# CityU-AIM-Group/SimT

Hardware: AMD Instinct MI355X
Metric: training images/sec at 768x768, DeepLabv2-R101+SimT (higher is better)
Workload: dtype bf16; 1 GPU; DeepLabv2-ResNet101 + SimT(C=19,K=3) full training iteration, batch=4/GPU, 768x768, bf16, 1xMI355X; global_batch=4, inputs=resident in HBM (see h2d_inclusive of a --full run for the PCIe-inclusive rate)

## Files before the change

### simt_amd/csrc/head_expand.hip

```cpp
#include "common.h"

struct TapArgs {
  const void* src;
  const float* bias;
  void* dst;
  int B, H, W, Q, QP, lds, ldd, ntaps;
  long M;
  short dy[SIMT_MAX_TAPS], dx[SIMT_MAX_TAPS];
};

__global__ __launch_bounds__(256) void tap_gather_sum_kernel(TapArgs a) {
  const int nq = a.QP >> 2;
  const long total = a.M * nq;
  const float* P = (const float*)a.src;
  float* y = (float*)a.dst;
  for (long idx = (long)blockIdx.x * blockDim.x + threadIdx.x; idx < total; idx += (long)gridDim.x * blockDim.x) {
    const int q = (int)(idx % nq);
    const long m = idx / nq;
    const int ox = (int)(m % a.W);
    const long t2 = m / a.W;
    const int oy = (int)(t2 % a.H);
    float4 acc = make_float4(0.f, 0.f, 0.f, 0.f);
    if (a.bias) {
      const int c = q * 4;
      acc.x = c + 0 < a.Q ? a.bias[c + 0] : 0.f;
      acc.y = c + 1 < a.Q ? a.bias[c + 1] : 0.f;
      acc.z = c + 2 < a.Q ? a.bias[c + 2] : 0.f;
      acc.w = c + 3 < a.Q ? a.bias[c + 3] : 0.f;
    }
    for (int t = 0; t < a.ntaps; ++t) {
      const int iy = oy + a.dy[t], ix = ox + a.dx[t];
      if (iy < 0 || iy >= a.H || ix < 0 || ix >= a.W) continue;
      const float4 v = *(const float4*)(P + (m + (long)a.dy[t] * a.W + a.dx[t]) * a.lds + t * a.QP + q * 4);
      acc.x += v.x; acc.y += v.y; acc.z += v.z; acc.w += v.w;
    }
    *(float4*)(y + m * a.ldd + q * 4) = acc;
  }
}

__global__ __launch_bounds__(256) void tap_scatter_kernel(TapArgs a) {
  const int ng = a.QP >> 3;
  const long total = a.M * a.ntaps * ng;
  const bf16_t* d = (const bf16_t*)a.src;
  bf16_t* G = (bf16_t*)a.dst;
  for (long idx = (long)blockIdx.x * blockDim.x + threadIdx.x; idx < total; idx += (long)gridDim.x * blockDim.x) {
    const int g = (int)(idx % ng);
    long r = idx / ng;
    const int t = (int)(r % a.ntaps);
    const long m = r / a.ntaps;
    const int ox = (int)(m % a.W);
    const int oy = (int)((m / a.W) % a.H);
    const int iy = oy - a.dy[t], ix = ox - a.dx[t];
    uint4 v = make_uint4(0u, 0u, 0u, 0u);
    if (iy >= 0 && iy < a.H && ix >= 0 && ix < a.W)
      v = *(const uint4*)(d + (m - ((long)a.dy[t] * a.W + a.dx[t])) * a.lds + g * 8);
    st_out16(G + m * a.ldd + t * a.QP + g * 8, v);
  }
}

static int tap_grid(long total) {
  long g = (total + 255) / 256;
  if (g > 256 * 16) g = 256 * 16;
  return (int)(g < 1 ? 1 : g);
}

extern "C" int simt_tap_gather_sum(const simt_tap_desc* d, simt_stream_t stream) {
  SIMT_CHECK(d && d->src && d->dst && d->ntaps >= 1 && d->ntaps <= SIMT_MAX_TAPS);
  SIMT_CHECK(d->QP % 4 == 0 && d->lds % 4 == 0 && d->ldd % 4 == 0 && d->QP <= d->ldd && d->ntaps * d->QP <= d->lds);
  TapArgs a;
  a.src = d->src; a.bias = d->bias; a.dst = d->dst; a.B = d->B; a.H = d->H; a.W = d->W; a.Q = d->Q; a.QP = d->QP;
  a.lds = d->lds; a.ldd = d->ldd; a.ntaps = d->ntaps; a.M = (long)d->B * d->H * d->W;
  for (int i = 0; i < SIMT_MAX_TAPS; ++i) { a.dy[i] = d->dy[i]; a.dx[i] = d->dx[i]; }
  hipLaunchKernelGGL(tap_gather_sum_kernel, dim3(tap_grid(a.M * (a.QP / 4))), dim3(256), 0, (hipStream_t)stream, a);
  SIMT_LAUNCH_CHECK();
  return SIMT_OK;
}

extern "C" int simt_tap_scatter(const simt_tap_desc* d, simt_stream_t stream) {
  SIMT_CHECK(d && d->src && d->dst && d->ntaps >= 1 && d->ntaps <= SIMT_MAX_TAPS);
  SIMT_CHECK(d->QP % 8 == 0 && d->lds % 8 == 0 && d->ldd % 8 == 0 && d->QP <= d->lds && d->ntaps * d->QP <= d->ldd);
  TapArgs a;
  a.src = d->src; a.bias = nullptr; a.dst = d->dst; a.B = d->B; a.H = d->H; a.W = d->W; a.Q = d->Q; a.QP = d->QP;
  a.lds = d->lds; a.ldd = d->ldd; a.ntaps = d->ntaps; a.M = (long)d->B * d->H * d->W;
  for (int i = 0; i < SIMT_MAX_TAPS; ++i) { a.dy[i] = d->dy[i]; a.dx[i] = d->dx[i]; }
  hipLaunchKernelGGL(tap_scatter_kernel, dim3(tap_grid(a.M * a.ntaps * (a.QP / 8))), dim3(256), 0, (hipStream_t)stream, a);
  SIMT_LAUNCH_CHECK();
  return SIMT_OK;
}
```

### simt_amd/step.py

```python
import ctypes as C
import math
import os

import numpy as np
import torch

from . import _lib as L
from . import ops
from . import trace
from .ema import EmaMixin
from .ema_teacher import TeacherMixin
from .engine import LaunchList, TrunkPlan, multi_heads, side_stream
from .online_labels import OnlineLabelMixin, check_balanced, check_settings
from .train_state import TrainStateMixin, state_sha256


class Hyper:

    def __init__(self, num_classes=19, open_classes=15, th_high=0.8, th_low=0.2, lambda_seg=0.1, lambda_place=0.1,
                 lambda_convex=0.5, lambda_volume=0.1, lambda_anchor=0.5, iter_size=1, lr=2.5e-4, lr_T=2.5e-4,
                 momentum=0.9, weight_decay=5e-4, power=0.9, num_steps=250000, skip_unapplied_grads=False):
        self.__dict__.update(locals())
        del self.__dict__["self"]


def lr_poly(base_lr, it, max_iter, power):
    return base_lr * ((1 - float(it) / max_iter) ** power)


def optim_listing(names, layers_root=("layer3", "layer4"), head_prefixes=("layer5", "layer6", "layer5_1", "layer6_1")):
    g0, g1 = {}, {}
    for n in names:
        root = n.split(".")[0]
        if root in layers_root:
            depth = len(n.split(".")) - 1
            g0[n] = depth
        elif root in head_prefixes:
            g1[n] = 1
    return g0, g1


def check_views(tr, teacher_image, fix_item, n):
    if not tr.teacher_view:
        if teacher_image is not None or fix_item is not None:
            raise ValueError("step(): teacher_image / fix_item need a trainer built with teacher_view=True")
        return [None] * n, [None] * n
    if teacher_image is None:
        raise ValueError("step(): this trainer was built with teacher_view=True and needs teacher_image (the frozen model's view)")
    teachers = list(teacher_image) if isinstance(teacher_image, (list, tuple)) else [teacher_image]
    maps = list(fix_item) if isinstance(fix_item, (list, tuple)) else [fix_item] * (n if fix_item is None else 1)
    if len(teachers) != n or len(maps) != n:
        raise ValueError(f"step() needs {n} teacher_image(s) and fix_item(s) (hp.iter_size), got {len(teachers)} and {len(maps)}")
    for t in teachers:
        if tuple(t.shape) != (tr.B, 3, tr.H, tr.W):
            raise ValueError(f"teacher_image of shape {tuple(t.shape)}, expected {(tr.B, 3, tr.H, tr.W)}")
    for m in maps:
        if m is not None and (tuple(m.shape) != (tr.B, tr.H, tr.W) or m.dtype != torch.uint8):
            raise ValueError(f"fix_item of shape {tuple(m.shape)} and dtype {m.dtype}, expected {(tr.B, tr.H, tr.W)} uint8")
    return teachers, maps


class SimTTrainer(TrainStateMixin, EmaMixin, TeacherMixin):
    def __init__(self, state, fixed_state, ntm1, ntm2, hp, class_dist, B, H, W, *, dtype=torch.bfloat16, device="cuda:0",
                 openset=True, process_group=None, w_init=None, layers=None, ema_decay=None, ema_teacher_every=None, teacher_view=False):
        self.hp, self.B, self.H, self.W, self.dtype = hp, B, H, W, dtype
        self.teacher_view = bool(teacher_view)
        dev = self.dev = torch.device(device)
        self.pg = process_group
        Cn, K = hp.num_classes, hp.open_classes
        self.C, self.Q = Cn, Cn + K
        f32 = torch.float32
        self.params = {k: v.detach().to(dev, f32 if v.dtype != torch.long else torch.long).clone() for k, v in state.items()}
        self.fixed_params = {k: v.detach().to(dev, f32 if v.dtype != torch.long else torch.long).clone()
                             for k, v in fixed_state.items()}
        self.frozen_sha256 = state_sha256(self.fixed_params)
        kw = {"layers": layers} if layers is not None else {}
        self.plan = TrunkPlan(self.params, B, H, W, multi_heads(Cn, K, openset), dtype=dtype, train=True,
                              grads_from_layer=3 if getattr(hp, "skip_unapplied_grads", False) else 0,
                              data_parallel=process_group is not None, **kw)
        self.fixed = TrunkPlan(self.fixed_params, B, H, W, multi_heads(Cn, 0, False), dtype=dtype, train=False,
                               stem_from=None if self.teacher_view else self.plan,
                               data_parallel=process_group is not None, **kw)
        assert self.plan.fwd_list.items[0].tag in ("simt_stem7_fwd", "simt_im2col_stem")
        assert self.plan.fwd_list.items[0].tag == "simt_im2col_stem" or self.plan.stem_desc.nsets == (1 if self.teacher_view else 2)
        assert not self.teacher_view or self.fixed.fwd_list.items[0].tag == self.plan.fwd_list.items[0].tag
        self._fwd_rest = LaunchList()
        self._fwd_rest.items = self.plan.fwd_list.items[1:]
        h, w = self.plan.heads[1].h, self.plan.heads[1].w
        self.h, self.w = h, w
        Q = self.Q
        self.ntm = [ntm1.detach().to(dev, f32).clone(), ntm2.detach().to(dev, f32).clone()]
        self._xchg = torch.zeros(16 + 2 * Q * Cn, device=dev)
        self._ntm_grad_flat = self._xchg[16:].view(2, Q, Cn)
        self.ntm_grad = [self._ntm_grad_flat[0], self._ntm_grad_flat[1]]
        self.ntm_m = [torch.zeros(Q, Cn, device=dev) for _ in range(2)]
        self.ntm_v = [torch.zeros(Q, Cn, device=dev) for _ in range(2)]
        wi = w_init if w_init is not None else torch.full((Q, Q), 1.0 / (Q - 1.0))
        self.wraw = [wi.detach().to(dev, f32).clone() for _ in range(2)]
        self.w_m = [torch.zeros(Q, Q, device=dev) for _ in range(2)]
        self.w_v = [torch.zeros(Q, Q, device=dev) for _ in range(2)]
        self.T = [torch.zeros(Q, Cn, device=dev) for _ in range(2)]
        self.cd = torch.as_tensor(np.asarray(class_dist), dtype=f32).to(dev)
        self.inner_steps = 10
        lib = L.load()
        self.nblk = lib.simt_head_nblk(B, H, W)
        self.part = torch.zeros(self.nblk, lib.simt_head_part_floats(Q, Cn), device=dev)
        self.keys = torch.zeros(lib.simt_head_keys_count(), device=dev, dtype=torch.int64)
        self.hout = torch.zeros(lib.simt_head_hout_floats(Q, Cn), device=dev)
        self.lout = self._xchg[:16]
        self._bad_reported = 0
        self.QP = ops.round_up(Q, 8)
        self.g1 = torch.zeros(2, B, H, w, self.QP, device=dev)
        self.ldf = self.fixed.ldp["x2"]
        self.fixp = torch.zeros(B * h * w, self.ldf, device=dev)
        self.label = torch.zeros(B, H, W, device=dev, dtype=torch.int64)
        hd = L.HeadDesc()
        p1, p2 = self.plan.out["x1"], self.plan.out["x2"]
        hd.pred1, hd.pred2, hd.fixp, hd.label = p1.data_ptr(), p2.data_ptr(), self.fixp.data_ptr(), self.label.data_ptr()
        hd.T1, hd.T2 = self.T[0].data_ptr(), self.T[1].data_ptr()
        hd.part, hd.keys, hd.hout, hd.g1 = self.part.data_ptr(), self.keys.data_ptr(), self.hout.data_ptr(), self.g1.data_ptr()
        hd.dpred1_f32, hd.dpred2_f32 = None, None
        d1, d2 = self.plan.dlogits["x1"], self.plan.dlogits["x2"]
        hd.dpred1_t, hd.dpred2_t = d1.data_ptr(), d2.data_ptr()
        hd.B, hd.h, hd.w, hd.H, hd.W, hd.C, hd.Q = B, h, w, H, W, Cn, Q
        hd.ldp, hd.ldf, hd.QP, hd.ld_f32, hd.ld_t = self.plan.ldp["x1"], self.ldf, self.QP, 0, d1.shape[1]
        hd.grad_dtype = ops.dt_code(dtype)
        hd.th_high, hd.th_low, hd.lambda_seg, hd.lambda_place = hp.th_high, hp.th_low, hp.lambda_seg, hp.lambda_place
        hd.gscale = 1.0 / hp.iter_size
        self.conf_label = torch.full((B, H, W), 255, device=dev, dtype=torch.uint8)
        hd.conf_out = self.conf_label.data_ptr()
        self._label_ws = torch.full((B, H, W), 255, device=dev, dtype=torch.uint8)
        hd.label_ws = self._label_ws.data_ptr()
        self.head_desc = hd
        self.fix_item = torch.zeros(B, H, W, device=dev, dtype=torch.uint8) if self.teacher_view else None
        self._fix_item_ptr = None
        ni = L.NtmInnerDesc()
        for k in range(2):
            ni.ntm[k], ni.w[k], ni.ntm_grad[k] = self.ntm[k].data_ptr(), self.wraw[k].data_ptr(), self.ntm_grad[k].data_ptr()
            ni.w_m[k], ni.w_v[k], ni.T_out[k] = self.w_m[k].data_ptr(), self.w_v[k].data_ptr(), self.T[k].data_ptr()
        ni.class_dist, ni.Q, ni.C, ni.steps = self.cd.data_ptr(), Q, Cn, self.inner_steps
        ni.beta1, ni.beta2, ni.eps = 0.9, 0.999, 1e-8
        self._skip_word = getattr(self.plan, "fbn_err", None)
        if self._skip_word is not None:
            ni.skip_if = self._skip_word.data_ptr()
        self.inner_desc = ni
        npd = L.NtmPostDesc()
        for k in range(2):
            npd.ntm[k], npd.w[k], npd.ntm_grad[k] = self.ntm[k].data_ptr(), self.wraw[k].data_ptr(), self.ntm_grad[k].data_ptr()
        npd.class_dist, npd.hout, npd.lout, npd.Q, npd.C = self.cd.data_ptr(), self.hout.data_ptr(), self.lout.data_ptr(), Q, Cn
        npd.lambda_seg, npd.lambda_convex, npd.lambda_volume = hp.lambda_seg, hp.lambda_convex, hp.lambda_volume
        npd.lambda_anchor, npd.gscale = hp.lambda_anchor, 1.0 / hp.iter_size
        self.post_desc = npd
        self._build_sgd()
        self.it_done = 0
        self._init_ema(ema_decay)
        self._init_teacher(ema_teacher_every)
        applied = [n for n in self.sgd_names if self.plan.grad_ready.get(n, 0) > 0]
        self._ev_post = None
        self._early_cut = max(self.plan.grad_ready[n] for n in applied) if applied else None
        if self._early_cut is not None:
            blk = min((m for m in self.plan.bwd_marks.values() if m[1] >= self._early_cut), key=lambda m: m[1], default=None)
            if blk is not None and blk[3] is not None:
                later = [c for c in sorted(set(self.plan.grad_ready.values())) if c >= blk[1]]
                self._early_cut = later[0] if later else None
        self._early_sgd = (os.environ.get("SIMT_EARLY_SGD", "1") != "0" and self._early_cut is not None
                           and hp.iter_size == 1 and self._early_cut < len(self.plan.bwd_list.items))
        self._pack_applied = self.plan.pack_subset(self.sgd_names) if self._early_sgd else None
        self._grad_acc = torch.zeros_like(self.plan.flat_grad) if hp.iter_size > 1 else None
        self.reducer = None
        if self.pg is not None:
            from .dp import BucketReducer, make_buckets
            order, sizes, end = self.exchange_table()
            be = int(float(os.environ.get("SIMT_DP_BUCKET_MB", "0")) * (1 << 18)) or self.BUCKET_ELEMS
            buckets = make_buckets(order, sizes, self.plan.grad_ready, bucket_elems=be)
            self.reducer = BucketReducer(self.plan.flat_grad[:end], buckets, group=self.pg, extra=[self._xchg[12:]])
            self.reducer.total_launches = len(self.plan.bwd_list.items)

    BUCKET_ELEMS = 8 << 20

    def exchange_table(self):
        sizes = {n: k for n, (_o, k) in self.plan.grad_offsets.items()}
        applied = set(self.sgd_names)
        order = [n for n in self.plan.grad_order if n in applied and self.plan.grad_ready.get(n, 0) > 0]
        assert order == self.plan.grad_order[:len(order)], "applied gradients must form a prefix of the flat buffer"
        return order, sizes, sum(sizes[n] for n in order)

    def _build_sgd(self, roots=("layer3", "layer4")):
        g0, g1 = optim_listing(self.plan.grads.keys(), layers_root=roots)
        recs = []
        self.mom = {}
        for group, listing in ((0, g0), (1, g1)):
            for n, mult in listing.items():
                p, g = self.params[n], self.plan.grads[n]
                buf = torch.zeros_like(p)
                self.mom[n] = buf
                recs.append((p.data_ptr(), g.data_ptr(), buf.data_ptr(), p.numel(), mult, group))
        self.sgd_names = list(g0) + list(g1)
        seg_dt = np.dtype([("p", "<u8"), ("g", "<u8"), ("buf", "<u8"), ("n", "<i8"), ("mult", "<i4"), ("group", "<i4")])
        segs = np.array(recs, dtype=seg_dt)
        chunk = 65536
        chunks = []
        for si, r in enumerate(recs):
            for ci in range((r[3] + chunk - 1) // chunk):
                chunks.append((si, ci))
        self.sgd_segs = torch.from_numpy(segs.view(np.uint8).copy()).to(self.dev)
        self.sgd_chunks = torch.tensor(chunks, dtype=torch.int32).to(self.dev)
        d = L.SgdDesc()
        d.segs, d.chunks, d.nchunks, d.chunk = self.sgd_segs.data_ptr(), self.sgd_chunks.data_ptr(), len(chunks), chunk
        d.momentum, d.dampening = self.hp.momentum, 0.0
        if getattr(self.plan, "fbn_err", None) is not None:
            d.skip_if = self.plan.fbn_err.data_ptr()
        self.sgd_desc = d

    def _micro_batch(self, image, label, st, teacher_image=None, fix_item=None):
        self.plan.x_in.copy_(image, non_blocking=True)
        self.label.copy_(label, non_blocking=True)
        if self.teacher_view:
            self.fixed.x_in.copy_(teacher_image, non_blocking=True)
            self._fix_item_ptr = None
            if fix_item is not None:
                self.fix_item.copy_(fix_item, non_blocking=True)
                self._fix_item_ptr = self.fix_item.data_ptr()
        head = self.plan.fwd_list.items[0]
        rc = head.fn(*head.args, st)
        if rc != 0:
            L.check(rc)
        main = torch.cuda.current_stream()
        side = side_stream(self.dev)
        ev_in = torch.cuda.Event()
        ev_in.record(main)
        with trace.range("forward"):
            self._fwd_rest.run()
        with torch.cuda.stream(side), trace.range("frozen-forward"):
            side.wait_event(ev_in)
            self.fixed.forward()
            ops.softmax_rows(self.fixed.out["x2"], self.ldf, self.fixp, self.ldf, self.B * self.h * self.w, self.C)
            ev_fix = torch.cuda.Event()
            ev_fix.record(side)
        main.wait_event(ev_fix)
        if self._ev_post is not None:
            main.wait_event(self._ev_post)
        with trace.range("head"):
            L.call("simt_head_loss_views", C.byref(self.head_desc), self._fix_item_ptr, st)
            ev_loss = torch.cuda.Event()
            ev_loss.record(main)
            with torch.cuda.stream(side):
                side.wait_event(ev_loss)
                L.call("simt_ntm_post", C.byref(self.post_desc), side.cuda_stream)
                self._ev_post = torch.cuda.Event()
                self._ev_post.record(side)
            L.call("simt_head_grad_views", C.byref(self.head_desc), self._fix_item_ptr, st)

    def step(self, image, label, it=None, teacher_image=None, fix_item=None):
        hp = self.hp
        teachers, maps = check_views(self, teacher_image, fix_item, hp.iter_size)
        it = self.it_done if it is None else it
        lr = lr_poly(hp.lr, it, hp.num_steps, hp.power)
        lr_T = lr_poly(hp.lr_T, it, hp.num_steps, hp.power)
        st = ops.stream_ptr()
        images = list(image) if isinstance(image, (list, tuple)) else [image]
        labels = list(label) if isinstance(label, (list, tuple)) else [label]
        if len(images) != hp.iter_size or len(labels) != hp.iter_size:
            raise ValueError(f"step() needs {hp.iter_size} micro-batch(es) (hp.iter_size), got {len(images)}")
        main, side = torch.cuda.current_stream(), side_stream(self.dev)
        ev0 = torch.cuda.Event()
        ev0.record(main)
        with torch.cuda.stream(side):
            side.wait_event(ev0)
            self._ntm_grad_flat.zero_()
            ni = self.inner_desc
            ni.step0, ni.lr = self.inner_steps * self.it_done, lr_T
            L.call("simt_ntm_inner_loop", C.byref(ni), side.cuda_stream)
        flat = self.plan.flat_grad
        for mi, (img, lab) in enumerate(zip(images, labels)):
            last = mi == hp.iter_size - 1
            self._micro_batch(img, lab, st, teachers[mi], maps[mi])
            if self._early_sgd:
                with trace.range("backward (+ exchange + early optimiser step)"):
                    self._backward_early_sgd(lr, st)
                continue
            if self.reducer is not None and hp.iter_size == 1:
                self.reducer.start()
                with trace.range("backward (+ bucketed exchange)"):
                    self.plan.backward(hook=self.reducer.ready_upto)
                torch.cuda.current_stream().wait_event(self._ev_post)
                with trace.range("exchange (flush + wait)"):
                    self.reducer.finish()
                continue
            with trace.range("backward"):
                self.plan.backward()
            if hp.iter_size > 1:
                if mi == 0:
                    self._grad_acc.copy_(flat)
                elif not last:
                    L.call("simt_vec_acc", self._grad_acc.data_ptr(), flat.data_ptr(), flat.numel(), 1, st)
                else:
                    L.call("simt_vec_acc", flat.data_ptr(), self._grad_acc.data_ptr(), flat.numel(), 1, st)
                    if self.reducer is not None:
                        torch.cuda.current_stream().wait_event(self._ev_post)
                        self.reducer.start()
                        self.reducer.finish()
        if not self._early_sgd:
            with trace.range("optimiser"):
                self._sgd(lr, st)
        torch.cuda.current_stream().wait_event(self._ev_post)
        for k in range(2):
            ops.adam_step(self.ntm[k], self.ntm_grad[k], self.ntm_m[k], self.ntm_v[k], lr=lr_T, step=self.it_done + 1, skip_if=self._skip_word)
        if not self._early_sgd:
            self.plan.repack()
            if self.ema is not None:
                self.ema.update(st)
                self._teacher_follows(st)
        self.it_done += 1
        return self.lout

    def _sgd(self, lr, st):
        d = self.sgd_desc
        d.lr[0], d.lr[1] = lr, lr * 10.0
        d.wd[0], d.wd[1] = self.hp.weight_decay, self.hp.weight_decay
        d.first_step = 1 if self.it_done == 0 else 0
        L.call("simt_sgd_multi", C.byref(d), st)

    def _backward_early_sgd(self, lr, st):
        main, side = torch.cuda.current_stream(), side_stream(self.dev)
        done = [False]
        red = self.reducer
        if red is not None:
            red.start()

        def hook(n, ev):
            if red is not None and not done[0]:
                red.ready_upto(n, ev)
            if done[0] or n < self._early_cut:
                return
            done[0] = True
            ev_main = torch.cuda.Event()
            ev_main.record(main)
            with torch.cuda.stream(side):
                side.wait_event(ev_main)
                if red is not None:
                    red.finish()
                self._sgd(lr, side.cuda_stream)
                self._pack_applied.run()
                if self.ema is not None:
                    self.ema.update(side.cuda_stream)
                    self._teacher_follows(side.cuda_stream)
        self.plan.backward(hook=hook)
        assert done[0]

    def state_dict(self):
        sd = {}
        for k, v in self.params.items():
            sd[k] = (v.detach().cpu() if not k.endswith("num_batches_tracked") else
                     torch.tensor(int(v.item()) + self._nbt_steps(k), dtype=torch.long))
        return sd

    def timed_lists(self):
        return [self.fixed.fwd_list, self.plan.fwd_list, self.plan.bwd_list]

    def losses(self):
        v = self.lout.cpu().tolist()
        self.plan.raise_on_fbn_error()
        bad = int(round(v[12] * (self.reducer.world if self.reducer is not None else 1))) - self._bad_reported
        self._bad_reported += max(bad, 0)
        if bad > 0:
            raise ValueError(f"{bad} label value(s) outside [0, {self.hp.num_classes}) that are not the ignore value 255")
        keys = ["total", "loss_p1", "loss_p2", "loss_y1", "loss_y2", "place", "convex", "volume", "anchor", "vol_ok"]
        return dict(zip(keys, v))


class WarmupTrainer(TrainStateMixin, EmaMixin, OnlineLabelMixin):

    def __init__(self, state, hp, B, H, W, *, dtype=torch.bfloat16, device="cuda:0", process_group=None, layers=None, ema_decay=None,
                 online_labels=None, online_labels_every=None, online_labels_balanced=None, online_labels_momentum=None):
        tau, every = check_settings(online_labels, online_labels_every, ema_decay)
        balanced = check_balanced(online_labels_balanced, online_labels_momentum, tau, hp.num_classes)
        self.hp, self.B, self.H, self.W, self.dtype = hp, B, H, W, dtype
        dev = self.dev = torch.device(device)
        self.pg = process_group
        Cn = self.C = hp.num_classes
        f32 = torch.float32
        self.params = {k: v.detach().to(dev, f32 if v.dtype != torch.long else torch.long).clone() for k, v in state.items()}
        kw = {"layers": layers} if layers is not None else {}
        self.plan = TrunkPlan(self.params, B, H, W, multi_heads(Cn, 0, False), dtype=dtype, train=True,
                              data_parallel=process_group is not None, **kw)
        h, w = self.h, self.w = self.plan.heads[1].h, self.plan.heads[1].w
        if tau is not None:
            self.fixed_params = {k: v.detach().to(dev, f32 if v.dtype != torch.long else torch.long).clone() for k, v in state.items()}
            self.frozen_sha256 = state_sha256(self.fixed_params)
            self.fixed = TrunkPlan(self.fixed_params, B, H, W, multi_heads(Cn, 0, False), dtype=dtype, train=False, stem_from=None,
                                   data_parallel=process_group is not None, **kw)
            self._fix_fwd = self.fixed.fwd_list
        lib = L.load()
        self.part = torch.zeros(lib.simt_head_nblk(B, H, W), lib.simt_head_part_floats(Cn, Cn), device=dev)
        self.keys = torch.zeros(lib.simt_head_keys_count(), device=dev, dtype=torch.int64)
        self.hout = torch.zeros(lib.simt_head_hout_floats(Cn, Cn), device=dev)
        self.bad_labels = torch.zeros(1, device=dev)
        self._bad_reported = 0
        self.QP = ops.round_up(Cn, 8)
        self.g1 = torch.zeros(2, B, H, w, self.QP, device=dev)
        self.label = torch.zeros(B, H, W, device=dev, dtype=torch.int64)
        hd = L.HeadDesc()
        d1, d2 = self.plan.dlogits["x1"], self.plan.dlogits["x2"]
        hd.pred1, hd.pred2, hd.fixp, hd.label = self.plan.out["x1"].data_ptr(), self.plan.out["x2"].data_ptr(), None, self.label.data_ptr()
        hd.T1, hd.T2 = None, None
        hd.part, hd.keys, hd.hout, hd.g1 = self.part.data_ptr(), self.keys.data_ptr(), self.hout.data_ptr(), self.g1.data_ptr()
        hd.dpred1_f32, hd.dpred2_f32, hd.dpred1_t, hd.dpred2_t = None, None, d1.data_ptr(), d2.data_ptr()
        hd.B, hd.h, hd.w, hd.H, hd.W, hd.C, hd.Q = B, h, w, H, W, Cn, Cn
        hd.ldp, hd.ldf, hd.QP, hd.ld_f32, hd.ld_t = self.plan.ldp["x1"], self.plan.ldp["x1"], self.QP, 0, d1.shape[1]
        hd.grad_dtype = ops.dt_code(dtype)
        hd.th_high, hd.th_low, hd.lambda_seg, hd.lambda_place, hd.gscale = 2.0, -1.0, hp.lambda_seg, 0.0, 1.0 / hp.iter_size
        hd.mode = 1
        self.head_desc = hd
        SimTTrainer._build_sgd(self, roots=("conv1", "layer1", "layer2", "layer3", "layer4"))
        self.it_done = 0
        self._init_ema(ema_decay)
        fix = (self.fixed.out["x2"], self.fixed.ldp["x2"]) if tau is not None else (None, 0)
        self._init_online(tau, every, *fix, 0, balanced)
        self.reducer = None
        if self.pg is not None:
            from .dp import BucketReducer, make_buckets
            sizes = {n: k for n, (_o, k) in self.plan.grad_offsets.items()}
            buckets = make_buckets(self.plan.grad_order, sizes, self.plan.grad_ready, bucket_elems=8 << 20)
            self.reducer = BucketReducer(self.plan.flat_grad, buckets, group=self.pg, extra=[self.bad_labels])
        self._grad_acc = None

    def step(self, image, label=None, it=None, teacher_image=None):
        hp = self.hp
        it = self.it_done if it is None else it
        lr = lr_poly(hp.lr, it, hp.num_steps, hp.power)
        st = ops.stream_ptr()
        images = list(image) if isinstance(image, (list, tuple)) else [image]
        labels, teachers = self._views(label, teacher_image, hp.iter_size)
        if len(images) != hp.iter_size or len(labels) != hp.iter_size:
            raise ValueError(f"step() needs {hp.iter_size} micro-batch(es) (hp.iter_size), got {len(images)}")
        flat = self.plan.flat_grad
        for mi, (img, lab) in enumerate(zip(images, labels)):
            self.plan.x_in.copy_(img, non_blocking=True)
            if self.online_labels is None:
                self.label.copy_(lab, non_blocking=True)
                self.plan.forward()
            else:
                ev_in = self._teacher_input(img, teachers[mi])
                self.plan.forward()
                self._teacher_labels(ev_in)
            L.call("simt_head_loss", C.byref(self.head_desc), st)
            L.call("simt_vec_acc", self.bad_labels.data_ptr(), self.hout.data_ptr() + 4 * 15, 1, 1, st)
            L.call("simt_head_grad", C.byref(self.head_desc), st)
            if self.reducer is not None and hp.iter_size == 1:
                self.reducer.start()
                self.plan.backward(hook=self.reducer.ready_upto)
                self.reducer.finish()
                continue
            self.plan.backward()
            if hp.iter_size > 1:
                if self._grad_acc is None:
                    self._grad_acc = torch.zeros_like(flat)
                if mi == 0:
                    self._grad_acc.copy_(flat)
                elif mi < hp.iter_size - 1:
                    L.call("simt_vec_acc", self._grad_acc.data_ptr(), flat.data_ptr(), flat.numel(), 1, st)
                else:
                    L.call("simt_vec_acc", flat.data_ptr(), self._grad_acc.data_ptr(), flat.numel(), 1, st)
                    if self.reducer is not None:
                        self.reducer.start()
                        self.reducer.finish()
        d = self.sgd_desc
        d.lr[0], d.lr[1] = lr, lr * 10.0
        d.wd[0], d.wd[1] = hp.weight_decay, hp.weight_decay
        d.first_step = 1 if self.it_done == 0 else 0
        L.call("simt_sgd_multi", C.byref(d), st)
        self.plan.repack()
        if self.ema is not None:
            self.ema.update(st)
            self._teacher_follows(st)
        self.it_done += 1
        return self.hout

    def state_dict(self):
        sd = {}
        for k, v in self.params.items():
            sd[k] = (v.detach().cpu() if not k.endswith("num_batches_tracked") else
                     torch.tensor(int(v.item()) + self._nbt_steps(k), dtype=torch.long))
        return sd

    def losses(self):
        v = torch.cat([self.hout[:16], self.bad_labels]).cpu().tolist()
        self.plan.raise_on_fbn_error()
        bad = int(round(v[16] * (self.reducer.world if self.reducer is not None else 1))) - self._bad_reported
        self._bad_reported += max(bad, 0)
        if bad > 0:
            raise ValueError(f"{bad} label value(s) outside [0, {self.hp.num_classes}) that are not the ignore value 255")
        return self._labelled({"total": v[14] / self.hp.iter_size, "loss_seg1": v[0], "loss_seg2": v[1]})
```

Before: 171.9 images/s.

## Drop unused frozen aux head and batch tap loads in gather-sum kernel

The frozen teacher network is now built without its auxiliary (layer3-level) head unless an environment variable asks for it, so that head's forward work is no longer run each step. Separately, the tap gather-sum kernel drops its grid-stride loop for one thread per output element at 128 threads per block, uses unsigned 32-bit index math, and issues up to nine tap loads at once before accumulating, so more memory requests are in flight. Out-of-bounds taps load from the thread's own row and are masked out rather than skipped. The risk is that something downstream may still read the frozen aux head output, and the size check now limits the gather to under 2^31 elements.

```diff
diff --git a/simt_amd/csrc/head_expand.hip b/simt_amd/csrc/head_expand.hip
--- a/simt_amd/csrc/head_expand.hip
+++ b/simt_amd/csrc/head_expand.hip
@@ -6,36 +6,46 @@
   void* dst;
   int B, H, W, Q, QP, lds, ldd, ntaps;
   long M;
-  short dy[SIMT_MAX_TAPS], dx[SIMT_MAX_TAPS];
+  int dy[SIMT_MAX_TAPS], dx[SIMT_MAX_TAPS];
 };
 
-__global__ __launch_bounds__(256) void tap_gather_sum_kernel(TapArgs a) {
-  const int nq = a.QP >> 2;
-  const long total = a.M * nq;
-  const float* P = (const float*)a.src;
-  float* y = (float*)a.dst;
-  for (long idx = (long)blockIdx.x * blockDim.x + threadIdx.x; idx < total; idx += (long)gridDim.x * blockDim.x) {
-    const int q = (int)(idx % nq);
-    const long m = idx / nq;
-    const int ox = (int)(m % a.W);
-    const long t2 = m / a.W;
-    const int oy = (int)(t2 % a.H);
-    float4 acc = make_float4(0.f, 0.f, 0.f, 0.f);
-    if (a.bias) {
-      const int c = q * 4;
-      acc.x = c + 0 < a.Q ? a.bias[c + 0] : 0.f;
-      acc.y = c + 1 < a.Q ? a.bias[c + 1] : 0.f;
-      acc.z = c + 2 < a.Q ? a.bias[c + 2] : 0.f;
-      acc.w = c + 3 < a.Q ? a.bias[c + 3] : 0.f;
+constexpr int TAP_BATCH = 9;
+__global__ __launch_bounds__(128) void tap_gather_sum_kernel(TapArgs a) {
+  const unsigned nq = (unsigned)a.QP >> 2;
+  const unsigned total = (unsigned)a.M * nq;
+  const unsigned idx = blockIdx.x * 128u + threadIdx.x;
+  if (idx >= total) return;
+  const unsigned m = idx / nq, q = idx - m * nq;
+  const unsigned t2 = m / (unsigned)a.W;
+  const int ox = (int)(m - t2 * (unsigned)a.W);
+  const int oy = (int)(t2 % (unsigned)a.H);
+  float4 acc = make_float4(0.f, 0.f, 0.f, 0.f);
+  if (a.bias) {
+    const int c = (int)q * 4;
+    acc.x = c + 0 < a.Q ? a.bias[c + 0] : 0.f;
+    acc.y = c + 1 < a.Q ? a.bias[c + 1] : 0.f;
+    acc.z = c + 2 < a.Q ? a.bias[c + 2] : 0.f;
+    acc.w = c + 3 < a.Q ? a.bias[c + 3] : 0.f;
+  }
+  const float* own = (const float*)a.src + (long)m * a.lds + q * 4;
+  for (int t0 = 0; t0 < a.ntaps; t0 += TAP_BATCH) {
+    float4 v[TAP_BATCH];
+    bool ok[TAP_BATCH];
+#pragma unroll
+    for (int j = 0; j < TAP_BATCH; ++j) {
+      const int t = min(t0 + j, SIMT_MAX_TAPS - 1);
+      const int dy = a.dy[t], dx = a.dx[t];
+      const int iy = oy + dy, ix = ox + dx;
+      ok[j] = t0 + j < a.ntaps && iy >= 0 && iy < a.H && ix >= 0 && ix < a.W;
+      const long off = ok[j] ? ((long)dy * a.W + dx) * a.lds + t * a.QP : 0l;
+      v[j] = *(const float4*)(own + off);
     }
-    for (int t = 0; t < a.ntaps; ++t) {
-      const int iy = oy + a.dy[t], ix = ox + a.dx[t];
-      if (iy < 0 || iy >= a.H || ix < 0 || ix >= a.W) continue;
-      const float4 v = *(const float4*)(P + (m + (long)a.dy[t] * a.W + a.dx[t]) * a.lds + t * a.QP + q * 4);
-      acc.x += v.x; acc.y += v.y; acc.z += v.z; acc.w += v.w;
+#pragma unroll
+    for (int j = 0; j < TAP_BATCH; ++j) {
+      if (ok[j]) { acc.x += v[j].x; acc.y += v[j].y; acc.z += v[j].z; acc.w += v[j].w; }
     }
-    *(float4*)(y + m * a.ldd + q * 4) = acc;
   }
+  *(float4*)((float*)a.dst + (long)m * a.ldd + q * 4) = acc;
 }
 
 __global__ __launch_bounds__(256) void tap_scatter_kernel(TapArgs a) {
@@ -71,7 +81,9 @@
   a.src = d->src; a.bias = d->bias; a.dst = d->dst; a.B = d->B; a.H = d->H; a.W = d->W; a.Q = d->Q; a.QP = d->QP;
   a.lds = d->lds; a.ldd = d->ldd; a.ntaps = d->ntaps; a.M = (long)d->B * d->H * d->W;
   for (int i = 0; i < SIMT_MAX_TAPS; ++i) { a.dy[i] = d->dy[i]; a.dx[i] = d->dx[i]; }
-  hipLaunchKernelGGL(tap_gather_sum_kernel, dim3(tap_grid(a.M * (a.QP / 4))), dim3(256), 0, (hipStream_t)stream, a);
+  const long total = a.M * (a.QP / 4);
+  SIMT_CHECK(total >= 0 && total < (1l << 31));
+  hipLaunchKernelGGL(tap_gather_sum_kernel, dim3((unsigned)(total > 128 ? (total + 127) / 128 : 1)), dim3(128), 0, (hipStream_t)stream, a);
   SIMT_LAUNCH_CHECK();
   return SIMT_OK;
 }
diff --git a/simt_amd/step.py b/simt_amd/step.py
--- a/simt_amd/step.py
+++ b/simt_amd/step.py
@@ -38,6 +38,11 @@
         elif root in head_prefixes:
             g1[n] = 1
     return g0, g1
+
+
+def frozen_heads(num_classes):
+    heads = multi_heads(num_classes, 0, False)
+    return heads if os.environ.get("SIMT_FROZEN_AUX_HEAD") == "1" else heads[1:]
 
 
 def check_views(tr, teacher_image, fix_item, n):
@@ -78,7 +83,7 @@
         self.plan = TrunkPlan(self.params, B, H, W, multi_heads(Cn, K, openset), dtype=dtype, train=True,
                               grads_from_layer=3 if getattr(hp, "skip_unapplied_grads", False) else 0,
                               data_parallel=process_group is not None, **kw)
-        self.fixed = TrunkPlan(self.fixed_params, B, H, W, multi_heads(Cn, 0, False), dtype=dtype, train=False,
+        self.fixed = TrunkPlan(self.fixed_params, B, H, W, frozen_heads(Cn), dtype=dtype, train=False,
                                stem_from=None if self.teacher_view else self.plan,
                                data_parallel=process_group is not None, **kw)
         assert self.plan.fwd_list.items[0].tag in ("simt_stem7_fwd", "simt_im2col_stem")
@@ -388,7 +393,7 @@
         if tau is not None:
             self.fixed_params = {k: v.detach().to(dev, f32 if v.dtype != torch.long else torch.long).clone() for k, v in state.items()}
             self.frozen_sha256 = state_sha256(self.fixed_params)
-            self.fixed = TrunkPlan(self.fixed_params, B, H, W, multi_heads(Cn, 0, False), dtype=dtype, train=False, stem_from=None,
+            self.fixed = TrunkPlan(self.fixed_params, B, H, W, frozen_heads(Cn), dtype=dtype, train=False, stem_from=None,
                                    data_parallel=process_group is not None, **kw)
             self._fix_fwd = self.fixed.fwd_list
         lib = L.load()
```

After: 172.3 images/s (median of 3 runs). No clear change (+0.2%).
